# 54rt1n/shardmerge

Measured on AMD Instinct MI355X. Metric: merged-weight GB/s per GPU + % HBM roofline, Llama-3-70B 3-way FFT merge, higher is better.
Workload: dtype f32; 1 GPU; Llama-3-70B block tensors, this rank's 1/8 slice (9 per block x 10 blocks), K=3 finetunes, bf16 in/out, resident in HBM; workload_id=llama3-70b-slice, k=3, parallelism=tensor-partition x1 (no data-path collective), streams_per_gpu=8

## Files before the change

shardmerge_amd/csrc/sm_capi.inc:

```

struct smhip_ctx {
    smhip::Pipeline<SM_BACKEND> pipe;
    explicit smhip_ctx(int device) : pipe(device) {}
};

#define SM_GUARD(ctx)                      \
    if (!(ctx)) return SMHIP_ERR_ARG;      \
    (ctx)->pipe.err.clear();
#define SM_FINISH(ctx, rc)                                                        \
    do {                                                                          \
        int rc__ = (rc);                                                          \
        if (rc__ == SMHIP_OK && !(ctx)->pipe.be.ok()) {                           \
            (ctx)->pipe.err = (ctx)->pipe.be.error();                             \
            rc__ = SMHIP_ERR_HIP;                                                 \
        }                                                                         \
        return rc__;                                                              \
    } while (0)

template <class Desc, class Scalars>
static int delta_tensor_check(smhip_ctx* ctx, const char* op, const Desc* d, const void* out, const float* delta_out,
                              bool need_base, Scalars scalars) {
    auto bad = [&](const char* what) { return ctx->pipe.fail(SMHIP_ERR_ARG, std::string(op) + ": " + what); };
    if (!d) return bad("null descriptor");
    if (d->k < 1 || d->k > SMHIP_MAX_MODELS) return bad("k out of range (1..16)");
// ... 293 lines not shown
    *norm_out = (float)out;
    SM_FINISH(ctx, SMHIP_OK);
}

int smhip_debug_option(smhip_ctx* ctx, const char* key, long value) {
    SM_GUARD(ctx);
    if (key && std::string(key) == "aten_overlap") { ctx->pipe.aten_overlap = value != 0; return SMHIP_OK; }
    if (key && std::string(key) == "emf_max_sample") { ctx->pipe.emf_max_sample = value >= 1 && value <= 4096 ? (int)value : smhip::EMF_MAX_SAMPLE; return SMHIP_OK; }
    if (key && std::string(key) == "aten_serial") { ctx->pipe.aten_serial = value != 0; return SMHIP_OK; }
    if (key && std::string(key) == "class_norms") { ctx->pipe.class_norms_mode = value >= 0 && value <= 2 ? (int)value : 1; return SMHIP_OK; }
    if (key && std::string(key) == "cand_cap") { ctx->pipe.debug_cand_cap = value > 0 ? (uint32_t)value : 0u; return SMHIP_OK; }
    if (key && std::string(key) == "sel_chunks") { ctx->pipe.debug_sel_chunks = value > 0 ? (uint32_t)value : 0u; return SMHIP_OK; }
    if (key && std::string(key) == "sel_flush_always") { ctx->pipe.debug_flush_always = value != 0; return SMHIP_OK; }
    if (key && std::string(key) == "fuse_norms") { ctx->pipe.fuse_norms = value != 0; return SMHIP_OK; }
    if (key && std::string(key) == "noise_seed") { ctx->pipe.noise_seed_base = (uint32_t)value; return SMHIP_OK; }
    if (key && std::string(key) == "spectral_intermediates") { ctx->pipe.spectral_inter = value != 0; return SMHIP_OK; }
    if (key && std::string(key) == "fuse_spec_norm") { ctx->pipe.fuse_spec_norm = value != 0; return SMHIP_OK; }
    if (key && std::string(key) == "sel_wgs_per_cu") { ctx->pipe.sel_wgs_per_cu = value > 0 ? (int)value : 5; return SMHIP_OK; }
    if (key && std::string(key) == "pair1d") { ctx->pipe.pair1d_enabled = value != 0; return SMHIP_OK; }
    if (key && std::string(key) == "spec_cull") { ctx->pipe.spec_cull = value != 0; return SMHIP_OK; }
    if (key && std::string(key) == "spec_min_bins") { ctx->pipe.spec_min_bins = value >= 0 ? (size_t)value : (size_t)1 << 20; return SMHIP_OK; }
    if (key && std::string(key) == "dftp_pairs") { ctx->pipe.dftp_pairs_enabled = value != 0; return SMHIP_OK; }
    if (key && std::string(key) == "f2s_pair") { ctx->pipe.f2s_pair = value != 0; return SMHIP_OK; }
    if (key && std::string(key) == "f1_multi") { ctx->pipe.f1_multi = value != 0; return SMHIP_OK; }
    if (key && std::string(key) == "force_bluestein") { ctx->pipe.debug_force_bluestein = value != 0; return SMHIP_OK; }
    if (key && std::string(key) == "force_split") { ctx->pipe.debug_force_split = value > 1 && value <= smhip::DFTP_MAX_P ? (int)value : 0; return SMHIP_OK; }
    if (key && std::string(key) == "fold_columns") { ctx->pipe.fold_enabled = value != 0; return SMHIP_OK; }
    if (key && std::string(key) == "fold_min_rows") { ctx->pipe.fold_min_rows = value > 0 ? (int)value : SM_FOLD_MIN_ROWS; return SMHIP_OK; }
    return ctx->pipe.fail(SMHIP_ERR_ARG, "unknown debug option");
}

int smhip_debug_query(smhip_ctx* ctx, const char* key, long* value) {
    SM_GUARD(ctx);
    if (!key || !value) return SMHIP_ERR_ARG;
    if (std::string(key) == "spec_hit") { *value = ctx->pipe.last_spec_verdict(); SM_FINISH(ctx, SMHIP_OK); }
    if (std::string(key) == "spec_checked" || std::string(key) == "spec_hits") {
        unsigned long long c = 0, h = 0;
        ctx->pipe.spec_totals(&c, &h);
        *value = (long)(std::string(key) == "spec_hits" ? h : c);
        SM_FINISH(ctx, SMHIP_OK);
    }
    if (std::string(key) == "aten_fast" || std::string(key) == "aten_group" || std::string(key) == "aten_slow") {
        unsigned long long v3[3];
        ctx->pipe.aten_stats(1, v3);
        *value = (long)v3[std::string(key) == "aten_fast" ? 0 : std::string(key) == "aten_group" ? 1 : 2];
        SM_FINISH(ctx, SMHIP_OK);
    }
    return ctx->pipe.fail(SMHIP_ERR_ARG, "unknown debug query");
}

int smhip_profile_enable(smhip_ctx* ctx, int on) { SM_GUARD(ctx); ctx->pipe.be.profile_enable(on != 0); return SMHIP_OK; }
int smhip_profile_reset(smhip_ctx* ctx) { SM_GUARD(ctx); ctx->pipe.be.profile_reset(); return SMHIP_OK; }
int smhip_profile_count(smhip_ctx* ctx) { return ctx ? ctx->pipe.be.profile_count() : 0; }
int smhip_profile_get(smhip_ctx* ctx, int i, const char** name, uint64_t* launches, double* total_ms) {
    SM_GUARD(ctx);
    return ctx->pipe.be.profile_get(i, name, launches, total_ms) ? SMHIP_OK : SMHIP_ERR_ARG;
}

}
```

shardmerge_amd/csrc/sm_kernels.hpp:

```cpp
#pragma once
#include <cmath>
#include <cstring>

#include "fft_engine.hpp"
#include "sm_aten_core.hpp"

namespace smhip {

struct cf4 { float x, y, z, w; };
struct u32x4 { uint32_t x, y, z, w; };

enum { DT_BF16 = 0, DT_F16 = 1, DT_F32 = 2 };

struct SigDesc {
    const void* x;
    const void* base;
    int dtype;
    float prescale;
};

SM_HD uint32_t umax(uint32_t a, uint32_t b) { return a > b ? a : b; }
SM_HD float u2f(uint32_t u) { float f; memcpy(&f, &u, 4); return f; }
SM_HD uint32_t f2u(float f) { uint32_t u; memcpy(&u, &f, 4); return u; }
SM_HD float bf16_to_f(uint32_t h) { return u2f(h << 16); }
// ... 1657 lines not shown
    unsigned long long rank;
    unsigned long long* hist;
    CandLists cand;
    int fuse_reduce;
    int sumsq;
    double* partials;
    int chunks;
    int flush_always;
    const uint32_t* skip;
    const float* blendB; float* blendR;
    const BlendConsts* consts; float t_sum;
    unsigned long long* hist1_out;
    const uint32_t* guess;
};

SM_HD float blend_slerp_one(const BlendConsts& c, float t_sum, float a, float b) {
    if (same_sign(a, b)) {
        if (fabsf(b) < c.thr) return a + t_sum * b;
        return a * c.cos_t + ((b - a * c.dot) * c.inv_rel) * c.sin_t;
    }
    return (fabsf(a) > fabsf(b)) ? a : b;
}

template <bool BLEND = false, class Ex>
SM_HD void k_select2(Ex& ex, const Select2Params& p) {
    typename Ex::template State<EmptyState> st;
    ex.init(st);
    uint32_t* lh = (uint32_t*)(ex.lds() + LDS_SCRATCH_FLOATS);
    uint32_t* lctl = lh + HIST_LO_BINS;
    uint32_t* lkeys = lctl + 8;
    cf4* lpairs = (cf4*)(lkeys + STAGE_KEYS);
    const int nt = ex.nthreads();
    const size_t total = (size_t)p.Cb * p.R;
    const size_t nquad = (total + 3) / 4;
    uint32_t* lh1 = lkeys + STAGE_KEYS;
    uint32_t prefix;
    BlendConsts bc;
    if constexpr (BLEND) {
        prefix = *p.guess - 1u;
        bc = *p.consts;
    } else {
        if (p.skip && *p.skip) return;
        wg_resolve(ex, st, p.hist1, HIST1_BINS, p.rank, (unsigned long long*)lkeys, lctl + 4);
        prefix = lctl[4];
        if (ex.bid() == 0) {
            ex.each(st, [&](int tid, EmptyState&) {
                if (tid == 0) {
// ... 7 lines not shown
    const WeightRanges wr = weight_ranges(p.R, p.C, p.Cb);
    ex.each(st, [&](int tid, EmptyState&) {
        for (int b = tid; b < HIST_LO_BINS; b += nt) lh[b] = 0;
        if (tid < 8) lctl[tid] = 0;
        if constexpr (BLEND) for (int b = tid; b < HIST1_BINS; b += nt) lh1[b] = 0;
    });
    ex.sync();
#ifndef SM_SEL_ROUND
#define SM_SEL_ROUND 16
#endif
#ifndef SM_SEL_U
#define SM_SEL_U 4
#endif
#ifndef SM_DIAG_SEL
#define SM_DIAG_SEL 0
#endif
    constexpr int ROUND = SM_SEL_ROUND;
    ex.each(st, [&](int, EmptyState& s) { s.red[0] = s.red[1] = s.red[2] = s.red[3] = 0.0; });
    for (int r0 = 0; r0 < p.chunks; r0 += ROUND) {
    const int r1 = (r0 + ROUND < p.chunks) ? r0 + ROUND : p.chunks;
    ex.each(st, [&](int tid, EmptyState& s) {
        double s00 = 0, s01 = 0, s11 = 0, cnt = 0;
        const size_t start = (size_t)ex.bid() * p.chunks * nt;
        const bool hasY = !BLEND && p.Y != nullptr;
        auto quad = [&](size_t i0, const float* a_in, const float* b, int n, bool uniform_w) {
            float q00 = 0.f, q01 = 0.f, q11 = 0.f, qc = 0.f;
            const uint32_t w0 = weight_at(wr, i0);
            float rr[4];
            const float* a = a_in;
            if constexpr (BLEND) {
#pragma unroll
                for (int e = 0; e < 4; ++e) rr[e] = blend_slerp_one(bc, p.t_sum, a_in[e], b[e]);
                if (n == 4 && uniform_w) { cf4 v = {rr[0], rr[1], rr[2], rr[3]}; *(cf4*)(p.blendR + i0) = v; }
                else for (int e = 0; e < n; ++e) p.blendR[i0 + e] = rr[e];
                a = rr;
            }
            const uint32_t lo = prefix << 20, hi = lo + (1u << 20);
            const bool has_hi = prefix < 2047u;
            uint32_t ka[4], kb[4], wv[4];
            bool hit = false;
#pragma unroll
            for (int e = 0; e < 4; ++e) {
                wv[e] = (e < n) ? (uniform_w ? w0 : weight_at(wr, i0 + e)) : 0u;
                ka[e] = f2u(a[e]) & 0x7fffffffu;
                kb[e] = hasY ? (f2u(b[e]) & 0x7fffffffu) : 0u;
                hit = hit || ((e < n) && ((ka[e] - lo) < (1u << 20) || (hasY && (kb[e] - lo) < (1u << 20))));
// ... 59 lines not shown
                if (hasY || BLEND) {
#pragma unroll
                    for (int u = 0; u < U; ++u) bv[u] = Y4[qv[u] < nquad ? qv[u] : nquad - 1];
                }
#pragma unroll
                for (int u = 0; u < U; ++u) {
                    if (c0 + u < r1 && qv[u] < nquad) {
                        const float a[4] = {av[u].x, av[u].y, av[u].z, av[u].w};
                        const float b[4] = {bv[u].x, bv[u].y, bv[u].z, bv[u].w};
                        quad(4 * qv[u], a, b, 4, !wr.full);
                    }
                }
            }
        } else {
            for (int c = r0; c < r1; ++c) {
                const size_t qi = start + (size_t)c * nt + tid;
                if (qi >= nquad) break;
                float a[4], b[4] = {0.f, 0.f, 0.f, 0.f};
                const int n = load_quad(p.X, 4 * qi, total, 0, a);
                if (hasY) load_quad(p.Y, 4 * qi, total, 0, b);
                if constexpr (BLEND) load_quad(p.blendB, 4 * qi, total, 0, b);
                quad(4 * qi, a, b, n, false);
            }
        }
        s.red[0] += s00; s.red[1] += s01; s.red[2] += s11; s.red[3] += cnt;
    });
    ex.sync();
    const bool last_round = r1 >= p.chunks;
    if (!last_round && !p.flush_always && lctl[0] <= (uint32_t)STAGE_KEYS / 2 && lctl[1] <= (uint32_t)STAGE_PAIRS / 2) continue;
    ex.each(st, [&](int tid, EmptyState&) {
        if (tid == 0) {
            uint32_t nk = lctl[0], np = lctl[1];
            bool over = false;
            if (nk > (uint32_t)STAGE_KEYS) { nk = STAGE_KEYS; over = true; }
            if (np > (uint32_t)STAGE_PAIRS) { np = STAGE_PAIRS; over = true; }
            const uint32_t bk = nk ? ex.global_atomic_add_ret_u32(&p.cand.counters[0], nk) : 0u;
            const uint32_t bp = np ? ex.global_atomic_add_ret_u32(&p.cand.counters[1], np) : 0u;
            if (bk + nk > p.cand.cap_keys || bp + np > p.cand.cap_pairs) over = true;
            if (over) { ex.global_atomic_or_u32(&p.cand.counters[2], 1u); if (!BLEND) ex.global_atomic_or_u32(&p.cand.counters[3], 1u); }
            lctl[0] = nk; lctl[1] = np; lctl[2] = bk; lctl[3] = bp;
        }
    });
    ex.sync();
    ex.each(st, [&](int tid, EmptyState&) {
        const uint32_t nk = lctl[0], np = lctl[1], bk = lctl[2], bp = lctl[3];
        for (uint32_t q = tid; q < nk; q += nt) if (bk + q < p.cand.cap_keys) p.cand.keys[bk + q] = lkeys[q];
// ... 710 lines not shown
            float qr = 0.f, qi2 = 0.f;
#pragma unroll
            for (int e = 0; e < 4; ++e) {
                if (e < n) {
                    const float w = (float)weight_at(wr, i0 + e);
                    if (!(fabsf(a[e]) < thr)) qr += w * a[e] * a[e];
                    qi2 += w * b[e] * b[e];
                }
            }
            sr += qr; si += qi2;
        }
        s.red[0] = sr; s.red[1] = si;
    });
    ex.template block_sum<2>(st, [&](const double* tot) {
        p.partials[2 * (size_t)ex.bid()] = tot[0];
        p.partials[2 * (size_t)ex.bid() + 1] = tot[1];
    });
}

SM_HD uint32_t hash_u32(uint32_t x) {
    x ^= x >> 16; x *= 0x7feb352du; x ^= x >> 15; x *= 0x846ca68bu; x ^= x >> 16;
    return x;
}
SM_HD float model_noise(uint32_t seed, size_t i, float sigma) {
    const uint32_t h1 = hash_u32((uint32_t)i * 2u + 1u + seed * 0x9e3779b9u) ^ hash_u32((uint32_t)(i >> 31) + seed);
    const uint32_t h2 = hash_u32(h1 + 0x68bc21ebu);
    if ((h2 >> 24) < 21u) return 0.f;
    const float s4 = (float)(h1 & 0xffffu) + (float)(h1 >> 16) + (float)(h2 & 0xffffu) + (float)(hash_u32(h2) >> 16);
    return sigma * 1.7320508f * (s4 * (1.0f / 65536.0f) - 2.0f);
}

struct SpecRescaleParams {
    const float* re; const float* im;
    float* dre; float* dim;
    int R, C, Cb;
    int vec4;
    float thr;
    float scale;
    float sigma; uint32_t seed;
    unsigned long long* hist;
    int chunks;
    double* im_partials;
};
template <class Ex>
SM_HD void k_spec_rescale(Ex& ex, const SpecRescaleParams& p) {
    typename Ex::template State<EmptyState> st;
    ex.init(st);
    uint32_t* lh = (uint32_t*)(ex.lds() + LDS_SCRATCH_FLOATS);
    const int nt = ex.nthreads();
    const size_t total = (size_t)p.Cb * p.R;
    const size_t nquad = (total + 3) / 4;
    const WeightRanges wr = weight_ranges(p.R, p.C, p.Cb);
    if (p.hist) {
        ex.each(st, [&](int tid, EmptyState&) { for (int b = tid; b < HIST1_BINS; b += nt) lh[b] = 0; });
        ex.sync();
    }
    ex.each(st, [&](int tid, EmptyState& s) {
        double imacc = 0.0;
        const size_t start = (size_t)ex.bid() * p.chunks * nt;
        for (int c = 0; c < p.chunks; ++c) {
            const size_t qi = start + (size_t)c * nt + tid;
            if (qi >= nquad) break;
            const size_t i0 = 4 * qi;
            float a[4], b[4] = {0.f, 0.f, 0.f, 0.f};
            const int n = load_quad(p.re, i0, total, p.vec4, a);
            if (p.im) load_quad(p.im, i0, total, p.vec4, b);
            float r[4], im[4];
#pragma unroll
            for (int e = 0; e < 4; ++e) {
                r[e] = (fabsf(a[e]) < p.thr) ? model_noise(p.seed, i0 + e, p.sigma) : a[e] * p.scale;
                im[e] = b[e] * p.scale;
            }
            if (p.vec4) {
                cf4 v = {r[0], r[1], r[2], r[3]};
                *(cf4*)(p.dre + i0) = v;
                if (p.im) { cf4 vi = {im[0], im[1], im[2], im[3]}; *(cf4*)(p.dim + i0) = vi; }
            } else {
                for (int e = 0; e < n; ++e) { p.dre[i0 + e] = r[e]; if (p.im) p.dim[i0 + e] = im[e]; }
            }
            if (p.hist) {
#pragma unroll
                for (int e = 0; e < 4; ++e)
// ... 1239 lines not shown
```

shardmerge_amd/csrc/sm_pipeline.hpp:

```cpp
#pragma once
#include <algorithm>
#include <cmath>
#include <cstdio>
#include <map>
#include <string>
#include <vector>

#include "../../include/shardmerge_hip.h"
#include "sm_kernels.hpp"
#include "sm_aten_norm.hpp"
#include "sm_bluestein.hpp"
#include "sm_lora.hpp"
#include "sm_ties.hpp"
#include "sm_dare.hpp"
#include "sm_breadcrumbs.hpp"
#include "sm_geo.hpp"

namespace smhip {

#define SM_KERNEL_TAG(Tag, ParamsT, NAME, CALL)                                      \
    struct Tag {                                                                     \
        using Params = ParamsT;                                                      \
        static constexpr int waves = 4;                                              \
        static constexpr int max_threads = 1024;                                     \
// ... 94 lines not shown
        found = true;
    }
}
inline bool plan_shape_static(int N, int& T, std::vector<int>& radices) {
    bool found = false;
#define SM_PLAN_FROM(...) plan_from_static<__VA_ARGS__>(N, T, radices, found);
    SM_STATIC_PLANS(SM_PLAN_FROM)
#undef SM_PLAN_FROM
    return found;
}

template <class PL>
inline bool plan_matches(const FftPlanDev& pl) {
    if (pl.N != PL::N || pl.T != PL::T || pl.npass != PL::npass || pl.lds_floats != PL::lds_floats || (pl.cx != 0) != PL::cx) return false;
    for (int i = 0; i < PL::npass; ++i)
        if (pl.radix[i] != PL::radix(i)) return false;
    return true;
}
SM_KERNEL_TAG(KF2R1, F2Params, "f2_cols_fwd", k_f2_r1(ex, p))
SM_KERNEL_TAG(KI1R1, I1Params, "i1_cols_inv", k_i1_r1(ex, p))
SM_KERNEL_TAG(KPublish, PublishParams, "publish", k_publish(ex, p))
SM_KERNEL_TAG(KHist, HistParams, "select_hist", k_hist(ex, p))
SM_KERNEL_TAG(KScan, ScanParams, "select_scan", k_scan(ex, p))
SM_KERNEL_TAG(KSelect2, Select2Params, "select_lvl2", k_select2<false>(ex, p))
SM_KERNEL_TAG(KSelect2Cull, Select2Params, "select_lvl2_cull", k_select2<false>(ex, p))
SM_KERNEL_TAG(KBlendSel, Select2Params, "blend", k_select2<true>(ex, p))
SM_KERNEL_TAG(KSpecCheck, SpecCheckParams, "select_spec_check", k_spec_check(ex, p))
SM_KERNEL_TAG(KSelect3, Select3Params, "select_lvl3_cand", k_select3(ex, p))
SM_KERNEL_TAG(KReduceCand, ReduceCandParams, "slerp_reduce_cand", k_reduce_cand(ex, p))
SM_KERNEL_TAG(KReduce, ReduceParams, "slerp_reduce", k_reduce(ex, p))
SM_KERNEL_TAG(KSlerpConsts, SlerpConstParams, "slerp_consts", k_slerp_consts(ex, p))
SM_KERNEL_TAG_LB(KClassEmf, ClassEmfParams, "class_norm_stats", k_class_emf(ex, p), 256, 2)
SM_KERNEL_TAG(KSumPartials, SumPartialsParams, "sum_partials", k_sum_partials(ex, p))
SM_KERNEL_TAG(KDeltaNorms, DeltaNormsParams, "delta_norms", k_delta_norms(ex, p))
SM_KERNEL_TAG(KSumPartialsN, SumNParams, "sum_partials", k_sum_partials_n(ex, p))
SM_KERNEL_TAG(KBlend, BlendParams, "blend", k_blend(ex, p))
SM_KERNEL_TAG(KCombine, CombineParams, "combine", k_combine(ex, p))
SM_KERNEL_TAG(KExpand, ExpandParams, "expand_full", k_expand(ex, p))
SM_KERNEL_TAG(KPack, PackParams, "pack_planes", k_pack(ex, p))
SM_KERNEL_TAG(KSplit, SplitParams, "split_complex", k_split(ex, p))
SM_KERNEL_TAG(KJoin, JoinParams, "join_complex", k_join(ex, p))
SM_KERNEL_TAG(KCull, CullParams, "cull_inplace", k_cull(ex, p))
SM_KERNEL_TAG(KAddition, AdditionParams, "addition_merge", k_addition(ex, p))
SM_KERNEL_TAG(KFnSums, FnSumsParams, "fn_slerp_sums", k_fn_sums(ex, p))
SM_KERNEL_TAG(KFnSlerpFin, FnSlerpFinParams, "fn_slerp_consts", k_fn_slerp_fin(ex, p))
SM_KERNEL_TAG(KFnSlerpRows0, FnSlerpRowsParams, "fn_slerp_relnorm", k_fn_slerp_rows<0>(ex, p))
SM_KERNEL_TAG(KFnSlerpRows1, FnSlerpRowsParams, "fn_slerp_out", k_fn_slerp_rows<1>(ex, p))
SM_KERNEL_TAG(KFnSlerpDen, FnSlerpDenParams, "fn_slerp_den", k_fn_slerp_den(ex, p))
SM_KERNEL_TAG(KSumsqAny, SumsqAnyParams, "fn_sumsq", k_sumsq_any(ex, p))
SM_KERNEL_TAG(KDivScalar, DivScalarParams, "fn_div_scalar", k_div_scalar(ex, p))
SM_KERNEL_TAG(KCorrPartial, CorrPartialParams, "correlate_pairs", k_corr_partial(ex, p))
SM_KERNEL_TAG(KCorrFinish, CorrFinishParams, "correlate_finish", k_corr_finish(ex, p))
SM_KERNEL_TAG(KSerialNorm, SerialNormParams, "serial_norm", k_serial_norm(ex, p))
SM_KERNEL_TAG(KSpecNorm, SpecNormParams, "spec_norm", k_spec_norm(ex, p))
SM_KERNEL_TAG(KSumsqCand, SumsqCandParams, "spec_norm_cand", k_sumsq_cand(ex, p))
SM_KERNEL_TAG(KSumSpec, SumSpecParams, "spec_norm_sum", k_sum_spec(ex, p))
SM_KERNEL_TAG(KSpecRescale, SpecRescaleParams, "spec_rescale", k_spec_rescale(ex, p))
SM_KERNEL_TAG(KDftp, DftpParams, "dft_across_slices", k_dftp(ex, p))
SM_KERNEL_TAG(KDftpPairs, DftpParams, "dft_across_slices", k_dftp_pairs(ex, p))
SM_KERNEL_TAG(KTranspose, TransposeParams, "transpose", k_transpose(ex, p))
SM_KERNEL_TAG_LB(KLoraPack, LoraPackParams, "lora_pack", k_lora_pack(ex, p), 256, 4)
SM_KERNEL_TAG_LB(KLoraBf16, LoraApplyParams, "lora_apply", k_lora_apply<DT_BF16>(ex, p), 256, 2)
SM_KERNEL_TAG_LB(KLoraF16, LoraApplyParams, "lora_apply", k_lora_apply<DT_F16>(ex, p), 256, 2)
SM_KERNEL_TAG_LB(KLoraF32, LoraApplyParams, "lora_apply", k_lora_apply<DT_F32>(ex, p), 256, 2)
SM_KERNEL_TAG_LB(KDoraNormBf16, LoraApplyParams, "dora_norm", k_dora_norm<DT_BF16>(ex, p), 256, 2)
SM_KERNEL_TAG_LB(KDoraNormF16, LoraApplyParams, "dora_norm", k_dora_norm<DT_F16>(ex, p), 256, 2)
SM_KERNEL_TAG_LB(KDoraNormF32, LoraApplyParams, "dora_norm", k_dora_norm<DT_F32>(ex, p), 256, 2)
SM_KERNEL_TAG_LB(KDoraScale, DoraScaleParams, "dora_scale", k_dora_scale(ex, p), DORA_SCALE_THREADS, 4)
SM_KERNEL_TAG_LB(KDoraApplyBf16, LoraApplyParams, "dora_apply", k_dora_apply<DT_BF16>(ex, p), 256, 2)
SM_KERNEL_TAG_LB(KDoraApplyF16, LoraApplyParams, "dora_apply", k_dora_apply<DT_F16>(ex, p), 256, 2)
SM_KERNEL_TAG_LB(KDoraApplyF32, LoraApplyParams, "dora_apply", k_dora_apply<DT_F32>(ex, p), 256, 2)
SM_KERNEL_TAG_LB(KTiesHist, TiesHistParams, "ties_hist", k_ties_hist(ex, p), 256, 4)
SM_KERNEL_TAG_LB(KTiesSelect, TiesSelectParams, "ties_select", k_ties_select(ex, p), TIES_SELECT_THREADS, 4)
SM_KERNEL_TAG_LB(KTiesMerge, TiesMergeParams, "ties_merge", k_ties_merge(ex, p), 256, 4)
SM_KERNEL_TAG_LB(KDareMerge, DareMergeParams, "dare_merge", k_dare_merge(ex, p), 256, 4)
SM_KERNEL_TAG_LB(KCrumbsHist, CrumbsHistParams, "crumbs_hist", k_crumbs_hist(ex, p), 256, 4)
SM_KERNEL_TAG_LB(KCrumbsSelect, CrumbsSelectParams, "crumbs_select", k_crumbs_select(ex, p), TIES_SELECT_THREADS, 4)
SM_KERNEL_TAG_LB(KCrumbsMerge, CrumbsMergeParams, "crumbs_merge", k_crumbs_merge(ex, p), 256, 4)
SM_KERNEL_TAG_LB(KGeoGram, GeoGramParams, "geo_gram", k_geo_gram<false>(ex, p), GEO_THREADS, 4)
SM_KERNEL_TAG_LB(KGeoGramTiled, GeoGramParams, "geo_gram", k_geo_gram<true>(ex, p), GEO_THREADS, 2)
SM_KERNEL_TAG_LB(KGeoFold, GeoFoldParams, "geo_gram_fold", k_geo_fold(ex, p), 256, 4)
SM_KERNEL_TAG_LB(KGeoCoef, GeoCoefParams, "geo_coef", k_geo_coef(ex, p), 256, 4)
SM_KERNEL_TAG_LB(KGeoCombine, GeoCombineParams, "geo_combine", k_geo_combine(ex, p), 256, 4)
SM_KERNEL_TAG_LB(KAtenPre, AtenPreParams, "aten_norm_pre", k_aten_pre<0>(ex, p), 256, 4)
SM_KERNEL_TAG_LB(KAtenPreC, AtenPreParams, "aten_norm_pre", k_aten_pre<1>(ex, p), 256, 4)
SM_KERNEL_TAG_LB(KAtenScan, AtenScanParams, "aten_norm_scan", k_aten_scan(ex, p), 256, 4)
SM_KERNEL_TAG_LB(KAtenRec, AtenRecParams, "aten_norm_rec", k_aten_rec(ex, p), 256, 4)
#ifndef SM_ATEN_PART_WAVES
#define SM_ATEN_PART_WAVES 3
#endif
SM_KERNEL_TAG_LB(KAtenPart16, AtenPartParams, "aten_norm_part", k_aten_part<ATEN_PART_RAW16>(ex, p), 256, SM_ATEN_PART_WAVES)
SM_KERNEL_TAG_LB(KAtenPart32, AtenPartParams, "aten_norm_part", k_aten_part<ATEN_PART_RAW32>(ex, p), 256, SM_ATEN_PART_WAVES)
SM_KERNEL_TAG_LB(KAtenPart, AtenPartParams, "aten_norm_part", k_aten_part<ATEN_PART_SIGNAL>(ex, p), 256, 2)
SM_KERNEL_TAG_LB(KAtenPartC, AtenPartParams, "aten_norm_part", k_aten_part<ATEN_PART_CLASS>(ex, p), 256, 2)
SM_KERNEL_TAG_LB(KAtenWalk, AtenWalkParams, "aten_norm_walk", k_aten_walk<0>(ex, p), 256, 4)
SM_KERNEL_TAG_LB(KAtenWalkC, AtenWalkParams, "aten_norm_walk", k_aten_walk<1>(ex, p), 256, 4)
SM_KERNEL_TAG_LB(KAtenFinish, AtenFinishParams, "aten_norm_finish", k_aten_finish(ex, p), 256, 4)
#define SM_SIDE_KERNELS_0(X) X(KAtenPre) X(KAtenPreC) X(KAtenScan) X(KAtenRec) X(KAtenPart16) X(KAtenPart32) X(KAtenPart) X(KAtenPartC) X(KAtenWalk) X(KAtenWalkC) X(KAtenFinish)
#define SM_SIDE_KERNELS_1(X) X(KF2R1) X(KI1R1) X(KPublish) X(KHist) X(KScan) X(KSelect2) X(KSelect2Cull) X(KBlendSel) \
    X(KSpecCheck) X(KSelect3) X(KReduceCand) X(KReduce) X(KSlerpConsts) X(KSumPartials) X(KClassEmf)
#define SM_SIDE_KERNELS_2(X) X(KDeltaNorms) X(KSumPartialsN) X(KBlend) X(KCombine) X(KExpand) X(KPack) X(KSplit) X(KJoin) \
    X(KCull) X(KAddition) X(KFnSums) X(KFnSlerpFin) X(KFnSlerpRows0) X(KFnSlerpRows1) X(KFnSlerpDen) X(KSumsqAny) X(KDivScalar) X(KCorrPartial) X(KCorrFinish) X(KSerialNorm) X(KSpecNorm) X(KSumsqCand) X(KSumSpec)       \
    X(KSpecRescale) X(KDftp) X(KDftpPairs) X(KTranspose) X(KLoraPack) X(KLoraBf16) X(KLoraF16) X(KLoraF32) \
    X(KDoraNormBf16) X(KDoraNormF16) X(KDoraNormF32) X(KDoraScale) X(KDoraApplyBf16) X(KDoraApplyF16) X(KDoraApplyF32)
#define SM_SIDE_KERNELS_7(X) X(KTiesHist) X(KTiesSelect) X(KTiesMerge) X(KDareMerge) X(KCrumbsHist) X(KCrumbsSelect) X(KCrumbsMerge) \
    X(KGeoGram) X(KGeoGramTiled) X(KGeoFold) X(KGeoCoef) X(KGeoCombine)
#define SM_SIDE_GROUPS 8

struct HostPlan {
    FftPlanDev dev;
    bool ok = false;
};

inline bool plan_radices(int N, int T, std::vector<int>& out) {
    out.clear();
    if (N == 1) { out.push_back(1); return true; }
    int rest = N, a = 0;
    while (rest % 2 == 0) { rest /= 2; ++a; }
    std::vector<int> odd;
    for (int p : {3, 5, 7, 11, 13})
        while (rest % p == 0) { rest /= p; odd.push_back(p); }
    if (rest != 1) return false;
    if (a > 0) {
        const int np = (a + 4) / 5;
        const int base = a / np, extra = a % np;
        for (int i = 0; i < np; ++i) out.push_back(1 << (base + (i < extra ? 1 : 0)));
// ... 64 lines not shown
    int ifft_policy = 1;
};

template <class B>
class Pipeline {
  public:
    B be;
    std::string err;
    void* stream = nullptr;
    uint32_t debug_cand_cap = 0;
    uint32_t debug_sel_chunks = 0;
    bool debug_flush_always = false;
    bool spec_cull = true;
    size_t spec_min_bins = 1 << 20;
    bool dftp_pairs_enabled = true;
    int debug_force_split = 0;
    int sel_wgs_per_cu = 5;
    bool safe_select = false;
    uint32_t noise_seed_base = 0;
    bool spectral_inter = true;
    bool f2s_pair = true;
    size_t f2s_pair_max_bins = (size_t)64 << 20;
    bool f1_multi = true;
    bool fuse_spec_norm = true;
    float noise_sigma = 1.2e-7f;

    explicit Pipeline(int device) : be(device) {}
    ~Pipeline() {
        for (auto& kv : plans_) if (kv.second.dev.tw) be.free((void*)kv.second.dev.tw);
        for (Buffer* b : {&cand_, &t1_, &small_, &tmpA_, &tmpB_, &tmpC_, &fullS_, &saveR_, &saveI_, &aten_, &emf_, &lora_, &dora_, &ties_}) if (b->p) be.free(b->p);
        for (Buffer& b : pool_) if (b.p) be.free(b.p);
        if (mail_) be.free_host(mail_);
        for (Buffer& b : inter_) if (b.p) be.free(b.p);
        for (Buffer& b : rowspec_) if (b.p) be.free(b.p);
        for (Buffer& b : tr_) if (b.p) be.free(b.p);
        for (auto& kv : rough_tw_) if (kv.second) be.free(kv.second);
        for (auto& kv : blue_) { if (kv.second.chirp) be.free(kv.second.chirp); if (kv.second.filt) be.free(kv.second.filt); }
    }

    int fail(int code, const std::string& msg) { err = msg; return code; }

    int get_plan(int N, FftPlanDev& out) {
        auto it = plans_.find(N);
        if (it == plans_.end()) {
            HostPlan hp;
            int T;
// ... 467 lines not shown
        SumPartialsParams sp;
        sp.partials = d_part(); sp.nparts = grid; sp.out = mail_->norm2;
        be.template launch<KSumPartials>(1, 1024, LDS_SCRATCH_FLOATS * 4, sp, stream);
        PublishParams pp;
        pp.flags = d_flags(); pp.thr = d_thr(0); pp.consts = d_consts(); pp.mail = mail_; pp.zero_flags = nullptr;
        be.template launch<KPublish>(1, 64, LDS_SCRATCH_FLOATS * 4, pp, stream);
        be.sync(stream);
        sre = mail_->norm2[0]; sim = mail_->norm2[1];
    }
    void run_spec_rescale(const Geo& g, const float* re, const float* im, float thr, float scale, bool role_a, bool hist,
                          int* im_parts = nullptr) {
        const size_t total = (size_t)g.Cb * g.R;
        SpecRescaleParams q;
        q.re = re; q.im = role_a ? im : nullptr;
        q.dre = plane(g, role_a ? P_REA : P_REB); q.dim = plane(g, P_IMA);
        q.R = g.R; q.C = g.Cw; q.Cb = g.Cb; q.vec4 = vec4(g);
        q.thr = thr; q.scale = scale; q.sigma = noise_sigma; q.seed = ++noise_seed_;
        q.hist = hist ? d_hist() : nullptr;
        q.chunks = pick_chunks((total + 3) / 4, 256, 8, 8);
        const int grid = stream_grid((total + 3) / 4, 256, q.chunks);
        const bool want_im = im_parts && role_a && (size_t)grid <= PART_IM_DOUBLES;
        if (im_parts) *im_parts = want_im ? grid : -1;
        q.im_partials = want_im ? d_part_im() : nullptr;
        be.template launch<KSpecRescale>(grid, 256, (LDS_SCRATCH_FLOATS + HIST1_BINS) * 4, q, stream);
    }
    void run_spec_norm_fused(int sel_parts, int im_parts, double& sre, double& sim) {
        SumsqCandParams sc;
        sc.cand = cand_lists(); sc.thr = d_thr(1); sc.partials = d_part() + 4 * (size_t)sel_parts;
        be.template launch<KSumsqCand>(CAND_GRID, 256, LDS_SCRATCH_FLOATS * 4, sc, stream);
        SumSpecParams sp;
        sp.part4 = d_part(); sp.n4 = sel_parts + CAND_GRID; sp.part1 = d_part_im(); sp.n1 = im_parts; sp.out = mail_->norm2;
        sp.zero_u32 = d_candctr(); sp.zero_u32_count = 3;
        be.template launch<KSumSpec>(1, 1024, LDS_SCRATCH_FLOATS * 4, sp, stream);
        PublishParams pp;
        pp.flags = d_flags(); pp.thr = d_thr(0); pp.consts = d_consts(); pp.mail = mail_; pp.zero_flags = nullptr;
        be.template launch<KPublish>(1, 64, LDS_SCRATCH_FLOATS * 4, pp, stream);
        be.sync(stream);
        sre = mail_->norm2[0]; sim = mail_->norm2[1];
    }

    void read_norms(int grid, double& na, double& nb) {
        SumPartialsParams sp;
        sp.partials = d_part(); sp.nparts = grid; sp.out = mail_->norm2;
        be.template launch<KSumPartials>(1, 1024, LDS_SCRATCH_FLOATS * 4, sp, stream);
        be.sync(stream);
        na = std::sqrt(mail_->norm2[0]); nb = std::sqrt(mail_->norm2[1]);
    }
// ... 18 lines not shown
            p.nsig = 2; p.swap = swap; p.scale[0] = scale0; p.scale[1] = scale1;
            p.reA = plane(g, P_REA); p.imA = plane(g, P_IMA); p.reB = plane(g, P_REB);
            p.hist = hist ? d_hist() : nullptr;
            const int binsq = f2_bins_host(p.plan);
            const int gridq = (int)round_up((size_t)(p.Cb + binsq - 1) / binsq, 64);
            const size_t ldsq = (LDS_SCRATCH_FLOATS + (size_t)2 * binsq * p.plan.lds_floats + HIST1_BINS) * 4;
            launch_fft<KF2Q>(p.plan, gridq, 2 * binsq * p.plan.T, ldsq, p);
            return SMHIP_OK;
        }
        p.t1 = (const cf4*)t1_.p; p.pitch4 = g.pitch4; p.ilv = g.ilv; p.R = g.R; p.C = g.C; p.Cb = g.C / 2 + 1;
        p.nsig = f2_nsig_for(p.plan.T);
        p.swap = swap; p.scale[0] = scale0; p.scale[1] = scale1;
        p.reA = plane(g, P_REA); p.imA = plane(g, P_IMA); p.reB = plane(g, P_REB);
        p.hist = hist ? d_hist() : nullptr;
        const int bins = p.nsig == 2 ? f2_bins_host(p.plan) : 1;
        const int ngroups = p.nsig == 2 ? 2 * bins : 1;
        const int grid = p.nsig == 2 ? (int)round_up((size_t)(p.Cb + bins - 1) / bins, 64) : (int)round_up((size_t)p.Cb * 2, 128);
        const size_t lds = (LDS_SCRATCH_FLOATS + (size_t)ngroups * p.plan.lds_floats + HIST1_BINS) * 4;
        if (g.batch > 1) { p.sl.wgs = grid; p.sl.t1_stride = g.t1_slice; p.sl.plane_stride = (size_t)(g.C / 2 + 1) * g.R; }
        launch_fft<KF2>(p.plan, grid * g.batch, ngroups * p.plan.T, lds, p);
        return SMHIP_OK;
    }

    static constexpr int CAND_GRID = 256;
    void run_select(const Geo& g, const float* X, const float* Y, unsigned long long rank, bool level1_done, float* thr_out,
                    bool fuse_reduce = false, int* nparts_out = nullptr, bool sumsq = false, int spec_slot = -1) {
        const size_t total = (size_t)g.Cb * g.R;
        HistParams h;
        h.X = X; h.Y = Y; h.R = g.R; h.C = g.Cw; h.Cb = g.Cb; h.vec4 = vec4(g); h.sel = d_sel(0);
        h.hist = d_hist(); h.chunks = pick_chunks((total + 3) / 4, 256, 8); h.only_if = nullptr;
        const int hgrid = stream_grid((total + 3) / 4, 256, h.chunks);
        const size_t hlds = (LDS_SCRATCH_FLOATS + HIST1_BINS) * 4;
        const size_t scan_lds = (LDS_SCRATCH_FLOATS + 2 * 256 + 32) * 4;
        ScanParams s;
        s.hist = d_hist(); s.sel = d_sel(0); s.value_out = thr_out; s.zero_also = nullptr; s.zero_count = 0;
        s.zero_u32 = nullptr; s.zero_u32_count = 0;
        if (!level1_done) { h.level = 1; be.template launch<KHist>(hgrid, 256, hlds, h, stream); }
        if (nparts_out) *nparts_out = 0;
        if (safe_select) {
            s.nbins = HIST1_BINS; s.shift = 11; s.final_level = 0; s.init = 1; s.rank_init = rank;
            be.template launch<KScan>(1, 256, scan_lds, s, stream);
            for (int level = 2; level <= 3; ++level) {
                h.level = level;
                be.template launch<KHist>(hgrid, 256, hlds, h, stream);
                s.nbins = HIST_LO_BINS; s.shift = 10; s.final_level = (level == 3); s.init = 0;
                be.template launch<KScan>(1, 256, scan_lds, s, stream);
            }
            return;
        }
        Select2Params q;
        q.X = X; q.Y = Y; q.R = g.R; q.C = g.Cw; q.Cb = g.Cb; q.vec4 = vec4(g); q.sel = d_sel(0);
        q.hist1 = d_hist(); q.rank = rank; q.hist = d_hist2();
        q.cand = cand_lists(); q.fuse_reduce = (fuse_reduce && Y) ? 1 : 0; q.partials = d_part();
        q.sumsq = (sumsq && !Y) ? 1 : 0;
        q.flush_always = debug_flush_always ? 1 : 0;
        q.chunks = debug_sel_chunks ? (int)debug_sel_chunks : pick_chunks((total + 3) / 4, 256, 8, sel_wgs_per_cu);
        int grid2 = stream_grid((total + 3) / 4, 256, q.chunks);
        while ((size_t)(grid2 + CAND_GRID) * 4 > PART_DOUBLES) { q.chunks *= 2; grid2 = stream_grid((total + 3) / 4, 256, q.chunks); }
        const size_t lds2 = (LDS_SCRATCH_FLOATS + HIST_LO_BINS + 8 + STAGE_KEYS) * 4 + (size_t)STAGE_PAIRS * sizeof(cf4);
        q.skip = nullptr; q.blendB = nullptr; q.blendR = nullptr; q.consts = nullptr; q.t_sum = 0.f; q.hist1_out = nullptr; q.guess = nullptr;
        if (spec_slot >= 0) {
            SpecCheckParams sc;
            sc.hist1 = d_hist(); sc.rank = rank; sc.guess = d_spec_guess(spec_slot); sc.flag = d_spec_flag();
            sc.sel = d_sel(0); sc.hist2 = d_hist2(); sc.counters = d_candctr();
            be.template launch<KSpecCheck>(1, 256, LDS_SCRATCH_FLOATS * 4 + (256 + 16) * 8 + 16, sc, stream);
            q.skip = d_spec_flag();
            be.template launch<KSelect2Cull>(grid2, 256, lds2, q, stream);
        } else {
            be.template launch<KSelect2>(grid2, 256, lds2, q, stream);
        }

        Select3Params t3;
        t3.cand = q.cand; t3.sel = d_sel(0); t3.hist2 = d_hist2(); t3.hist = d_hist3();
        be.template launch<KSelect3>(CAND_GRID, 256, (LDS_SCRATCH_FLOATS + HIST_LO_BINS + 8 + 2 * 256 + 32) * 4, t3, stream);

        s.hist = d_hist3(); s.sel = d_sel(1); s.nbins = HIST_LO_BINS; s.shift = 10; s.final_level = 1; s.init = 0;
        s.zero_also = d_hist(); s.zero_count = HIST1_BINS + HIST_LO_BINS;
        if (!q.fuse_reduce && !q.sumsq) { s.zero_u32 = d_candctr(); s.zero_u32_count = 3; }
        be.template launch<KScan>(1, 256, scan_lds, s, stream);

        if (q.sumsq && nparts_out) *nparts_out = grid2;
        if (q.fuse_reduce) {
            ReduceCandParams rc;
            rc.cand = q.cand; rc.thr = thr_out; rc.partials = d_part() + 4 * (size_t)grid2;
            be.template launch<KReduceCand>(CAND_GRID, 256, LDS_SCRATCH_FLOATS * 4, rc, stream);
            if (nparts_out) *nparts_out = grid2 + CAND_GRID;
        }
    }

    void run_blend(const Geo& g, int mode, int agreement, float t, float t_sum, bool hist) {
        const size_t total = (size_t)g.Cb * g.R;
        BlendParams b;
        b.reA = plane(g, P_REA); b.reB = plane(g, P_REB); b.reR = plane(g, P_RER);
        b.R = g.R; b.C = g.Cw; b.Cb = g.Cb; b.vec4 = vec4(g);
        b.mode = mode; b.agreement = agreement; b.t = t; b.t_sum = t_sum;
        b.consts = d_consts(); b.hist = hist ? d_hist() : nullptr; b.chunks = pick_chunks((total + 3) / 4, 256, 8, 8);
        be.template launch<KBlend>(stream_grid((total + 3) / 4, 256, b.chunks), 256, (LDS_SCRATCH_FLOATS + HIST1_BINS) * 4, b, stream);
    }

    void run_blend_spec(const Geo& g, float t_sum, bool sumsq, int spec_slot) {
        const size_t total = (size_t)g.Cb * g.R;
        Select2Params q;
        q.X = plane(g, P_REA); q.Y = nullptr; q.R = g.R; q.C = g.Cw; q.Cb = g.Cb; q.vec4 = vec4(g); q.sel = d_sel(0);
        q.hist1 = nullptr; q.rank = 0; q.hist = d_hist2();
        q.cand = cand_lists(); q.fuse_reduce = 0; q.partials = d_part(); q.sumsq = sumsq ? 1 : 0;
        q.flush_always = debug_flush_always ? 1 : 0;
        q.chunks = cull_select_chunks(total);
        q.skip = nullptr;
        q.blendB = plane(g, P_REB); q.blendR = plane(g, P_RER); q.consts = d_consts(); q.t_sum = t_sum;
        q.hist1_out = d_hist(); q.guess = d_spec_guess(spec_slot);
        const int grid = stream_grid((total + 3) / 4, 256, q.chunks);
        const size_t lds = (LDS_SCRATCH_FLOATS + HIST_LO_BINS + 8 + STAGE_KEYS + HIST1_BINS) * 4;
        be.template launch<KBlendSel>(grid, 256, lds, q, stream);
    }
    long last_spec_verdict() {
        if (!small_.p) return -1;
        uint32_t v = 0;
        be.d2h(&v, d_spec_flag(), sizeof v, stream);
        be.sync(stream);
        return (long)v;
    }
    void spec_totals(unsigned long long* checked, unsigned long long* hits) {
        uint32_t v[3] = {0, 0, 0};
        if (small_.p) { be.d2h(v, d_spec_flag(), sizeof v, stream); be.sync(stream); }
        *checked = v[1]; *hits = v[2];
    }
    int cull_select_chunks(size_t total) const {
        int chunks = debug_sel_chunks ? (int)debug_sel_chunks : pick_chunks((total + 3) / 4, 256, 8, sel_wgs_per_cu);
        int grid2 = stream_grid((total + 3) / 4, 256, chunks);
        while ((size_t)(grid2 + CAND_GRID) * 4 > PART_DOUBLES) { chunks *= 2; grid2 = stream_grid((total + 3) / 4, 256, chunks); }
        return chunks;
    }

    void run_slerp_consts(const Geo& g, bool have_thr, float t, int fused_parts, const float* ref_norms = nullptr,
                          const double* emf_part = nullptr, int emf_nparts = 0, int emf_elo = 0) {
        const size_t total = (size_t)g.Cb * g.R;
// ... 1675 lines not shown
```

Baseline: 86.82 GB/s.

## Add specialized vec4 unrolled streaming paths for select and spectral rescale kernels

Adds compile-time mode specializations of the level-2 select/blend kernel (keys-only, sumsq, fused pair) and the spectral rescale kernel (role A/B). Each specialization uses unrolled vec4 loads with clamped indices and no per-element generic branching. The noise hash high part is hoisted out of the loop when indices fit in 32 bits. The goal is to cut branch and instruction overhead in these memory-bound streaming passes. In exchange it adds more kernel instantiations and a stream_v1 switch that falls back to the old path.

```diff
diff --git a/shardmerge_amd/csrc/sm_capi.inc b/shardmerge_amd/csrc/sm_capi.inc
--- a/shardmerge_amd/csrc/sm_capi.inc
+++ b/shardmerge_amd/csrc/sm_capi.inc
@@ -339,6 +339,7 @@
     if (key && std::string(key) == "spec_min_bins") { ctx->pipe.spec_min_bins = value >= 0 ? (size_t)value : (size_t)1 << 20; return SMHIP_OK; }
     if (key && std::string(key) == "dftp_pairs") { ctx->pipe.dftp_pairs_enabled = value != 0; return SMHIP_OK; }
     if (key && std::string(key) == "f2s_pair") { ctx->pipe.f2s_pair = value != 0; return SMHIP_OK; }
+    if (key && std::string(key) == "stream_v1") { ctx->pipe.stream_v1 = value != 0; return SMHIP_OK; }
     if (key && std::string(key) == "f1_multi") { ctx->pipe.f1_multi = value != 0; return SMHIP_OK; }
     if (key && std::string(key) == "force_bluestein") { ctx->pipe.debug_force_bluestein = value != 0; return SMHIP_OK; }
     if (key && std::string(key) == "force_split") { ctx->pipe.debug_force_split = value > 1 && value <= smhip::DFTP_MAX_P ? (int)value : 0; return SMHIP_OK; }
@@ -357,6 +358,8 @@
         *value = (long)(std::string(key) == "spec_hits" ? h : c);
         SM_FINISH(ctx, SMHIP_OK);
     }
+    if (std::string(key) == "rescale_role_a") { *value = (long)ctx->pipe.rescale_role_a; return SMHIP_OK; }
+    if (std::string(key) == "rescale_im_sums") { *value = (long)ctx->pipe.rescale_im_sums; return SMHIP_OK; }
     if (std::string(key) == "aten_fast" || std::string(key) == "aten_group" || std::string(key) == "aten_slow") {
         unsigned long long v3[3];
         ctx->pipe.aten_stats(1, v3);
diff --git a/shardmerge_amd/csrc/sm_kernels.hpp b/shardmerge_amd/csrc/sm_kernels.hpp
--- a/shardmerge_amd/csrc/sm_kernels.hpp
+++ b/shardmerge_amd/csrc/sm_kernels.hpp
@@ -1703,7 +1703,20 @@
     return (fabsf(a) > fabsf(b)) ? a : b;
 }
 
-template <bool BLEND = false, class Ex>
+enum {
+    SEL_GENERIC = 0,
+    SEL_KEYS = 1,
+    SEL_SUMSQ = 2,
+    SEL_FUSED = 3,
+};
+SM_HD float mul_add(float a, float b, float c) {
+#if defined(__HIP_DEVICE_COMPILE__)
+    return __builtin_fmaf(a, b, c);
+#else
+    return a * b + c;
+#endif
+}
+template <bool BLEND = false, int MODE = SEL_GENERIC, class Ex>
 SM_HD void k_select2(Ex& ex, const Select2Params& p) {
     typename Ex::template State<EmptyState> st;
     ex.init(st);
@@ -1757,6 +1770,109 @@
     ex.each(st, [&](int tid, EmptyState& s) {
         double s00 = 0, s01 = 0, s11 = 0, cnt = 0;
         const size_t start = (size_t)ex.bid() * p.chunks * nt;
+        if constexpr (MODE != SEL_GENERIC) {
+        constexpr bool HASY = MODE == SEL_FUSED;
+        const uint32_t lo = prefix << 20, hi = lo + (1u << 20);
+        const bool has_hi = prefix < 2047u;
+        const bool hi_num = has_hi && hi <= 0x7f800000u;
+        const uint32_t hspan = 0x7f800000u - hi;
+        auto squad = [&](size_t i0, const float* a_in, const float* b) {
+            float q00 = 0.f, q01 = 0.f, q11 = 0.f, qc = 0.f;
+            const uint32_t w = weight_at(wr, i0);
+            const float wf = (float)w;
+            float rr[4];
+            const float* a = a_in;
+            if constexpr (BLEND) {
+#pragma unroll
+                for (int e = 0; e < 4; ++e) rr[e] = blend_slerp_one(bc, p.t_sum, a_in[e], b[e]);
+                cf4 v = {rr[0], rr[1], rr[2], rr[3]};
+                *(cf4*)(p.blendR + i0) = v;
+                a = rr;
+            }
+            uint32_t ka[4], kb[4];
+            bool hit = false;
+#pragma unroll
+            for (int e = 0; e < 4; ++e) {
+                ka[e] = f2u(a[e]) & 0x7fffffffu;
+                hit = hit || (ka[e] - lo) < (1u << 20);
+                if constexpr (HASY) {
+                    kb[e] = f2u(b[e]) & 0x7fffffffu;
+                    hit = hit || (kb[e] - lo) < (1u << 20);
+                }
+            }
+            if constexpr (BLEND) {
+#pragma unroll
+                for (int e = 0; e < 4; ++e) ex.lds_atomic_add(&lh1[ka[e] >> 20], w);
+            }
+            if (hit && !(SM_DIAG_SEL & 1)) {
+#pragma unroll
+                for (int e = 0; e < 4; ++e) {
+                    if ((ka[e] - lo) < (1u << 20)) {
+                        ex.lds_atomic_add(&lh[(ka[e] >> 10) & 1023u], w);
+                        const uint32_t pos = ex.lds_atomic_add_ret(&lctl[0], 1u);
+                        if (pos < (uint32_t)STAGE_KEYS) lkeys[pos] = ka[e] | ((w - 1u) << 31);
+                    }
+                    if constexpr (HASY) {
+                        if ((kb[e] - lo) < (1u << 20)) {
+                            ex.lds_atomic_add(&lh[(kb[e] >> 10) & 1023u], w);
+                            const uint32_t pos = ex.lds_atomic_add_ret(&lctl[0], 1u);
+                            if (pos < (uint32_t)STAGE_KEYS) lkeys[pos] = kb[e] | ((w - 1u) << 31);
+                            if (same_sign(a[e], b[e])) {
+                                const uint32_t pp = ex.lds_atomic_add_ret(&lctl[1], 1u);
+                                if (pp < (uint32_t)STAGE_PAIRS) { cf4 v = {a[e], b[e], wf, 0.f}; lpairs[pp] = v; }
+                            }
+                        }
+                    }
+                }
+            }
+            if constexpr (MODE == SEL_SUMSQ) {
+#pragma unroll
+                for (int e = 0; e < 4; ++e) {
+                    const bool in = has_hi && ka[e] >= hi;
+                    const float av = in ? a[e] : 0.f;
+                    q00 = mul_add(wf * av, av, q00);
+                }
+                s00 += q00;
+            }
+            if constexpr (MODE == SEL_FUSED) {
+                if (!(SM_DIAG_SEL & 2)) {
+#pragma unroll
+                    for (int e = 0; e < 4; ++e) {
+                        const bool in = hi_num && (kb[e] - hi) <= hspan && (ka[e] - 1u) < 0x7f800000u
+                                        && (int32_t)(f2u(a[e]) ^ f2u(b[e])) >= 0;
+                        const float av = in ? a[e] : 0.f, bv = in ? b[e] : 0.f;
+                        const float wa = wf * av;
+                        q00 = mul_add(wa, av, q00); q01 = mul_add(wa, bv, q01); q11 = mul_add(wf * bv, bv, q11); qc += in ? wf : 0.f;
+                    }
+                }
+                s00 += q00; s01 += q01; s11 += q11; cnt += qc;
+            }
+        };
+        constexpr int U = SM_SEL_U;
+        const cf4* X4 = (const cf4*)p.X;
+        const cf4* Y4 = (const cf4*)(BLEND ? p.blendB : p.Y);
+        for (int c0 = r0; c0 < r1; c0 += U) {
+            cf4 av[U], bv[U];
+            size_t qv[U];
+#pragma unroll
+            for (int u = 0; u < U; ++u) {
+                qv[u] = start + (size_t)(c0 + u) * nt + tid;
+                av[u] = X4[qv[u] < nquad ? qv[u] : nquad - 1];
+            }
+            if constexpr (HASY || BLEND) {
+#pragma unroll
+                for (int u = 0; u < U; ++u) bv[u] = Y4[qv[u] < nquad ? qv[u] : nquad - 1];
+            }
+#pragma unroll
+            for (int u = 0; u < U; ++u) {
+                if (c0 + u < r1 && qv[u] < nquad) {
+                    const float a[4] = {av[u].x, av[u].y, av[u].z, av[u].w};
+                    const float b[4] = {bv[u].x, bv[u].y, bv[u].z, bv[u].w};
+                    squad(4 * qv[u], a, b);
+                }
+            }
+        }
+        } else {
         const bool hasY = !BLEND && p.Y != nullptr;
         auto quad = [&](size_t i0, const float* a_in, const float* b, int n, bool uniform_w) {
             float q00 = 0.f, q01 = 0.f, q11 = 0.f, qc = 0.f;
@@ -1862,6 +1978,7 @@
                 if constexpr (BLEND) load_quad(p.blendB, 4 * qi, total, 0, b);
                 quad(4 * qi, a, b, n, false);
             }
+        }
         }
         s.red[0] += s00; s.red[1] += s01; s.red[2] += s11; s.red[3] += cnt;
     });
@@ -2618,12 +2735,15 @@
     x ^= x >> 16; x *= 0x7feb352du; x ^= x >> 15; x *= 0x846ca68bu; x ^= x >> 16;
     return x;
 }
-SM_HD float model_noise(uint32_t seed, size_t i, float sigma) {
-    const uint32_t h1 = hash_u32((uint32_t)i * 2u + 1u + seed * 0x9e3779b9u) ^ hash_u32((uint32_t)(i >> 31) + seed);
+SM_HD float model_noise_hi(uint32_t seed, size_t i, float sigma, uint32_t hhi) {
+    const uint32_t h1 = hash_u32((uint32_t)i * 2u + 1u + seed * 0x9e3779b9u) ^ hhi;
     const uint32_t h2 = hash_u32(h1 + 0x68bc21ebu);
     if ((h2 >> 24) < 21u) return 0.f;
     const float s4 = (float)(h1 & 0xffffu) + (float)(h1 >> 16) + (float)(h2 & 0xffffu) + (float)(hash_u32(h2) >> 16);
     return sigma * 1.7320508f * (s4 * (1.0f / 65536.0f) - 2.0f);
+}
+SM_HD float model_noise(uint32_t seed, size_t i, float sigma) {
+    return model_noise_hi(seed, i, sigma, hash_u32((uint32_t)(i >> 31) + seed));
 }
 
 struct SpecRescaleParams {
@@ -2638,7 +2758,11 @@
     int chunks;
     double* im_partials;
 };
-template <class Ex>
+enum { RESC_GENERIC = 0, RESC_B = 1, RESC_A = 2 };
+#ifndef SM_RESC_U
+#define SM_RESC_U 2
+#endif
+template <int MODE = RESC_GENERIC, class Ex>
 SM_HD void k_spec_rescale(Ex& ex, const SpecRescaleParams& p) {
     typename Ex::template State<EmptyState> st;
     ex.init(st);
@@ -2654,6 +2778,62 @@
     ex.each(st, [&](int tid, EmptyState& s) {
         double imacc = 0.0;
         const size_t start = (size_t)ex.bid() * p.chunks * nt;
+        if constexpr (MODE != RESC_GENERIC) {
+        constexpr int U = SM_RESC_U;
+        constexpr bool ROLE_A = MODE == RESC_A;
+        const cf4* re4 = (const cf4*)p.re;
+        const cf4* im4 = (const cf4*)p.im;
+        const bool low_index = total <= ((size_t)1 << 31);
+        const uint32_t hhi0 = hash_u32(p.seed);
+        for (int c0 = 0; c0 < p.chunks; c0 += U) {
+            cf4 av[U], bv[U];
+            size_t qv[U];
+#pragma unroll
+            for (int u = 0; u < U; ++u) {
+                qv[u] = start + (size_t)(c0 + u) * nt + tid;
+                av[u] = re4[qv[u] < nquad ? qv[u] : nquad - 1];
+            }
+            if constexpr (ROLE_A) {
+#pragma unroll
+                for (int u = 0; u < U; ++u) bv[u] = im4[qv[u] < nquad ? qv[u] : nquad - 1];
+            }
+#pragma unroll
+            for (int u = 0; u < U; ++u) {
+                if (c0 + u < p.chunks && qv[u] < nquad) {
+                    const size_t i0 = 4 * qv[u];
+                    const float a[4] = {av[u].x, av[u].y, av[u].z, av[u].w};
+                    uint32_t hhi = hhi0;
+                    if (!low_index) hhi = hash_u32((uint32_t)(i0 >> 31) + p.seed);
+                    float r[4];
+#pragma unroll
+                    for (int e = 0; e < 4; ++e)
+                        r[e] = (fabsf(a[e]) < p.thr) ? model_noise_hi(p.seed, i0 + e, p.sigma, hhi) : a[e] * p.scale;
+                    cf4 v = {r[0], r[1], r[2], r[3]};
+                    *(cf4*)(p.dre + i0) = v;
+                    const uint32_t w = weight_at(wr, i0);
+                    if (p.hist) {
+#pragma unroll
+                        for (int e = 0; e < 4; ++e) ex.lds_atomic_add(&lh[(f2u(r[e]) & 0x7fffffffu) >> 20], w);
+                    }
+                    if constexpr (ROLE_A) {
+                        const float b[4] = {bv[u].x, bv[u].y, bv[u].z, bv[u].w};
+                        float im[4];
+#pragma unroll
+                        for (int e = 0; e < 4; ++e) im[e] = b[e] * p.scale;
+                        cf4 vi = {im[0], im[1], im[2], im[3]};
+                        *(cf4*)(p.dim + i0) = vi;
+                        if (p.im_partials) {
+                            const float wf = (float)w;
+                            float q = 0.f;
+#pragma unroll
+                            for (int e = 0; e < 4; ++e) q = mul_add(wf * im[e], im[e], q);
+                            imacc += q;
+                        }
+                    }
+                }
+            }
+        }
+        } else
         for (int c = 0; c < p.chunks; ++c) {
             const size_t qi = start + (size_t)c * nt + tid;
             if (qi >= nquad) break;
diff --git a/shardmerge_amd/csrc/sm_pipeline.hpp b/shardmerge_amd/csrc/sm_pipeline.hpp
--- a/shardmerge_amd/csrc/sm_pipeline.hpp
+++ b/shardmerge_amd/csrc/sm_pipeline.hpp
@@ -140,9 +140,17 @@
 SM_KERNEL_TAG(KPublish, PublishParams, "publish", k_publish(ex, p))
 SM_KERNEL_TAG(KHist, HistParams, "select_hist", k_hist(ex, p))
 SM_KERNEL_TAG(KScan, ScanParams, "select_scan", k_scan(ex, p))
-SM_KERNEL_TAG(KSelect2, Select2Params, "select_lvl2", k_select2<false>(ex, p))
-SM_KERNEL_TAG(KSelect2Cull, Select2Params, "select_lvl2_cull", k_select2<false>(ex, p))
-SM_KERNEL_TAG(KBlendSel, Select2Params, "blend", k_select2<true>(ex, p))
+#define SM_MODE_KERNEL_TAG(Tag, ParamsT, NAME, CALL)                                 \
+    template <int M> struct Tag {                                                    \
+        using Params = ParamsT;                                                      \
+        static constexpr int waves = 4;                                              \
+        static constexpr int max_threads = 1024;                                     \
+        static const char* name() { return NAME; }                                   \
+        template <class Ex> static SM_HD void run(Ex& ex, const Params& p) { CALL; } \
+    };
+SM_MODE_KERNEL_TAG(KSelect2, Select2Params, "select_lvl2", (k_select2<false, M>(ex, p)))
+SM_MODE_KERNEL_TAG(KSelect2Cull, Select2Params, "select_lvl2_cull", (k_select2<false, M>(ex, p)))
+SM_MODE_KERNEL_TAG(KBlendSel, Select2Params, "blend", (k_select2<true, M>(ex, p)))
 SM_KERNEL_TAG(KSpecCheck, SpecCheckParams, "select_spec_check", k_spec_check(ex, p))
 SM_KERNEL_TAG(KSelect3, Select3Params, "select_lvl3_cand", k_select3(ex, p))
 SM_KERNEL_TAG(KReduceCand, ReduceCandParams, "slerp_reduce_cand", k_reduce_cand(ex, p))
@@ -173,7 +181,7 @@
 SM_KERNEL_TAG(KSpecNorm, SpecNormParams, "spec_norm", k_spec_norm(ex, p))
 SM_KERNEL_TAG(KSumsqCand, SumsqCandParams, "spec_norm_cand", k_sumsq_cand(ex, p))
 SM_KERNEL_TAG(KSumSpec, SumSpecParams, "spec_norm_sum", k_sum_spec(ex, p))
-SM_KERNEL_TAG(KSpecRescale, SpecRescaleParams, "spec_rescale", k_spec_rescale(ex, p))
+SM_MODE_KERNEL_TAG(KSpecRescale, SpecRescaleParams, "spec_rescale", k_spec_rescale<M>(ex, p))
 SM_KERNEL_TAG(KDftp, DftpParams, "dft_across_slices", k_dftp(ex, p))
 SM_KERNEL_TAG(KDftpPairs, DftpParams, "dft_across_slices", k_dftp_pairs(ex, p))
 SM_KERNEL_TAG(KTranspose, TransposeParams, "transpose", k_transpose(ex, p))
@@ -215,11 +223,12 @@
 SM_KERNEL_TAG_LB(KAtenWalkC, AtenWalkParams, "aten_norm_walk", k_aten_walk<1>(ex, p), 256, 4)
 SM_KERNEL_TAG_LB(KAtenFinish, AtenFinishParams, "aten_norm_finish", k_aten_finish(ex, p), 256, 4)
 #define SM_SIDE_KERNELS_0(X) X(KAtenPre) X(KAtenPreC) X(KAtenScan) X(KAtenRec) X(KAtenPart16) X(KAtenPart32) X(KAtenPart) X(KAtenPartC) X(KAtenWalk) X(KAtenWalkC) X(KAtenFinish)
-#define SM_SIDE_KERNELS_1(X) X(KF2R1) X(KI1R1) X(KPublish) X(KHist) X(KScan) X(KSelect2) X(KSelect2Cull) X(KBlendSel) \
+#define SM_SIDE_KERNELS_1(X) X(KF2R1) X(KI1R1) X(KPublish) X(KHist) X(KScan) X(KSelect2<SEL_GENERIC>) X(KSelect2<SEL_KEYS>) X(KSelect2<SEL_SUMSQ>) X(KSelect2<SEL_FUSED>) \
+    X(KSelect2Cull<SEL_GENERIC>) X(KSelect2Cull<SEL_KEYS>) X(KSelect2Cull<SEL_SUMSQ>) X(KBlendSel<SEL_GENERIC>) X(KBlendSel<SEL_KEYS>) X(KBlendSel<SEL_SUMSQ>) \
     X(KSpecCheck) X(KSelect3) X(KReduceCand) X(KReduce) X(KSlerpConsts) X(KSumPartials) X(KClassEmf)
 #define SM_SIDE_KERNELS_2(X) X(KDeltaNorms) X(KSumPartialsN) X(KBlend) X(KCombine) X(KExpand) X(KPack) X(KSplit) X(KJoin) \
     X(KCull) X(KAddition) X(KFnSums) X(KFnSlerpFin) X(KFnSlerpRows0) X(KFnSlerpRows1) X(KFnSlerpDen) X(KSumsqAny) X(KDivScalar) X(KCorrPartial) X(KCorrFinish) X(KSerialNorm) X(KSpecNorm) X(KSumsqCand) X(KSumSpec)       \
-    X(KSpecRescale) X(KDftp) X(KDftpPairs) X(KTranspose) X(KLoraPack) X(KLoraBf16) X(KLoraF16) X(KLoraF32) \
+    X(KSpecRescale<RESC_GENERIC>) X(KSpecRescale<RESC_B>) X(KSpecRescale<RESC_A>) X(KDftp) X(KDftpPairs) X(KTranspose) X(KLoraPack) X(KLoraBf16) X(KLoraF16) X(KLoraF32) \
     X(KDoraNormBf16) X(KDoraNormF16) X(KDoraNormF32) X(KDoraScale) X(KDoraApplyBf16) X(KDoraApplyF16) X(KDoraApplyF32)
 #define SM_SIDE_KERNELS_7(X) X(KTiesHist) X(KTiesSelect) X(KTiesMerge) X(KDareMerge) X(KCrumbsHist) X(KCrumbsSelect) X(KCrumbsMerge) \
     X(KGeoGram) X(KGeoGramTiled) X(KGeoFold) X(KGeoCoef) X(KGeoCombine)
@@ -330,6 +339,8 @@
     bool f2s_pair = true;
     size_t f2s_pair_max_bins = (size_t)64 << 20;
     bool f1_multi = true;
+    bool stream_v1 = false;
+    unsigned long long rescale_role_a = 0, rescale_im_sums = 0;
     bool fuse_spec_norm = true;
     float noise_sigma = 1.2e-7f;
 
@@ -843,7 +854,12 @@
         const bool want_im = im_parts && role_a && (size_t)grid <= PART_IM_DOUBLES;
         if (im_parts) *im_parts = want_im ? grid : -1;
         q.im_partials = want_im ? d_part_im() : nullptr;
-        be.template launch<KSpecRescale>(grid, 256, (LDS_SCRATCH_FLOATS + HIST1_BINS) * 4, q, stream);
+        if (role_a) ++rescale_role_a;
+        if (want_im) ++rescale_im_sums;
+        const size_t lds = (LDS_SCRATCH_FLOATS + HIST1_BINS) * 4;
+        if (stream_v1 || !q.vec4 || q.C < 0) be.template launch<KSpecRescale<RESC_GENERIC>>(grid, 256, lds, q, stream);
+        else if (q.im) be.template launch<KSpecRescale<RESC_A>>(grid, 256, lds, q, stream);
+        else be.template launch<KSpecRescale<RESC_B>>(grid, 256, lds, q, stream);
     }
     void run_spec_norm_fused(int sel_parts, int im_parts, double& sre, double& sim) {
         SumsqCandParams sc;
@@ -908,6 +924,11 @@
         return SMHIP_OK;
     }
 
+    int select_mode(const Select2Params& q) const {
+        if (stream_v1 || !q.vec4 || q.C < 0) return SEL_GENERIC;
+        if (q.Y) return q.fuse_reduce ? SEL_FUSED : SEL_GENERIC;
+        return q.sumsq ? SEL_SUMSQ : SEL_KEYS;
+    }
     static constexpr int CAND_GRID = 256;
     void run_select(const Geo& g, const float* X, const float* Y, unsigned long long rank, bool level1_done, float* thr_out,
                     bool fuse_reduce = false, int* nparts_out = nullptr, bool sumsq = false, int spec_slot = -1) {
@@ -951,9 +972,18 @@
             sc.sel = d_sel(0); sc.hist2 = d_hist2(); sc.counters = d_candctr();
             be.template launch<KSpecCheck>(1, 256, LDS_SCRATCH_FLOATS * 4 + (256 + 16) * 8 + 16, sc, stream);
             q.skip = d_spec_flag();
-            be.template launch<KSelect2Cull>(grid2, 256, lds2, q, stream);
+            switch (q.Y ? SEL_GENERIC : select_mode(q)) {
+                case SEL_KEYS: be.template launch<KSelect2Cull<SEL_KEYS>>(grid2, 256, lds2, q, stream); break;
+                case SEL_SUMSQ: be.template launch<KSelect2Cull<SEL_SUMSQ>>(grid2, 256, lds2, q, stream); break;
+                default: be.template launch<KSelect2Cull<SEL_GENERIC>>(grid2, 256, lds2, q, stream);
+            }
         } else {
-            be.template launch<KSelect2>(grid2, 256, lds2, q, stream);
+            switch (select_mode(q)) {
+                case SEL_KEYS: be.template launch<KSelect2<SEL_KEYS>>(grid2, 256, lds2, q, stream); break;
+                case SEL_SUMSQ: be.template launch<KSelect2<SEL_SUMSQ>>(grid2, 256, lds2, q, stream); break;
+                case SEL_FUSED: be.template launch<KSelect2<SEL_FUSED>>(grid2, 256, lds2, q, stream); break;
+                default: be.template launch<KSelect2<SEL_GENERIC>>(grid2, 256, lds2, q, stream);
+            }
         }
 
         Select3Params t3;
@@ -997,7 +1027,11 @@
         q.hist1_out = d_hist(); q.guess = d_spec_guess(spec_slot);
         const int grid = stream_grid((total + 3) / 4, 256, q.chunks);
         const size_t lds = (LDS_SCRATCH_FLOATS + HIST_LO_BINS + 8 + STAGE_KEYS + HIST1_BINS) * 4;
-        be.template launch<KBlendSel>(grid, 256, lds, q, stream);
+        switch (select_mode(q)) {
+            case SEL_KEYS: be.template launch<KBlendSel<SEL_KEYS>>(grid, 256, lds, q, stream); break;
+            case SEL_SUMSQ: be.template launch<KBlendSel<SEL_SUMSQ>>(grid, 256, lds, q, stream); break;
+            default: be.template launch<KBlendSel<SEL_GENERIC>>(grid, 256, lds, q, stream);
+        }
     }
     long last_spec_verdict() {
         if (!small_.p) return -1;
```

Measured after the change: 86.09 GB/s. About the same (-0.8%).
